# kjedrzejewski/video-cycle_gan-upscaling

Measured on AMD Instinct MI355X. Metric: upscaled frames/s (train step, G+D fwd+bwd) at 256->512, higher is better.
Workload: dtype f32; 1 GPU; C2: make_upscaler_orig((512,512,3),k=3,x2,res=9) + PatchGAN-70, batch 8/GPU, gan2 wiring, Wasserstein + pixel-MSE, faithful 3-call step incl. predict pass; global_batch=8, frame=256x256->512x512, parallelism=dp1, launch=hipGraph replay

## Files before the change

video-cycle_gan-upscaling_amd/csrc/conv_transpose.hip:

```cpp
#include "vcg_common.hpp"
#include <type_traits>

namespace {

struct ConvTParams {
    const float* x;
    const float* w;
    float* y;
    const float* bias;
    const float* prelu;
    const float* residual;
    int n, cin, h, w_, cout, oh, ow;
    int tiles_x, tiles_y, co_blocks;
    int act;
    float alpha;
};

constexpr int phase_of(int k, int cb) { return (((k - cb) % 2) + 2) % 2; }
constexpr int d_of(int k, int cb) { return (k - cb - phase_of(k, cb)) / 2; }
constexpr int dmin_of(int K, int cb) { int m = 1000; for (int k = 0; k < K; ++k) m = d_of(k, cb) < m ? d_of(k, cb) : m; return m; }
constexpr int dmax_of(int K, int cb) { int m = -1000; for (int k = 0; k < K; ++k) m = d_of(k, cb) > m ? d_of(k, cb) : m; return m; }

template <int K, int CBY, int CBX, int CK, int MT>
struct ConvTCfg {
    static constexpr int QROWS = 4;
    static constexpr int DMINY = dmin_of(K, CBY), DMAXY = dmax_of(K, CBY);
    static constexpr int DMINX = dmin_of(K, CBX), DMAXX = dmax_of(K, CBX);
    static constexpr int NDY = DMAXY - DMINY + 1, NDX = DMAXX - DMINX + 1;
    static constexpr int NR = QROWS + DMAXY - DMINY;
    static constexpr int NC = 32 + DMAXX - DMINX;
    static constexpr int PLANE = NR * NC;
    static constexpr int T = K * K;
    static constexpr int IN_ELEMS = CK * PLANE;
    static constexpr int MB = 32 * MT;
    static constexpr int W_ELEMS = CK * T * MB;
    static constexpr int IN_PT = (IN_ELEMS + 255) / 256;
    static constexpr int W_PT = (W_ELEMS + 255) / 256;
    static constexpr size_t LDS_BYTES = (size_t)(IN_ELEMS + W_ELEMS) * sizeof(float);
};

template <int K, int CBY, int CBX, int CK, int MT>
__global__ __launch_bounds__(256, (MT == 1 ? 2 : 1)) void convt_kernel(const ConvTParams p) {
    using C = ConvTCfg<K, CBY, CBX, CK, MT>;
    extern __shared__ __attribute__((aligned(16))) float smem[];
    float* s_in = smem;
    float* s_w = smem + C::IN_ELEMS;

    const int tid = threadIdx.x, lane = tid & 63, wv = tid >> 6;
    const int half = lane >> 5, l31 = lane & 31;
    int b = blockIdx.x;
    const int cb = b % p.co_blocks; b /= p.co_blocks;
    const int tx = b % p.tiles_x;   b /= p.tiles_x;
    const int ty = b % p.tiles_y;   b /= p.tiles_y;
    const int n = b;
    const int qx0 = tx * 32, qy0 = ty * C::QROWS, co0 = cb * C::MB;
    const int gy0 = qy0 - C::DMAXY, gx0 = qx0 - C::DMAXX;
    const float* xn = p.x + (size_t)n * p.cin * p.h * p.w_;

    float rin[C::IN_PT], rw[C::W_PT];
    unsigned in_off[C::IN_PT];
#pragma unroll
    for (int i = 0; i < C::IN_PT; ++i) {
        const int e = tid + i * 256;
        unsigned off = VCG_OOB;
        if (e < C::IN_ELEMS) {
            const int ci = e / C::PLANE, rem = e % C::PLANE;
            const int r = rem / C::NC, c = rem % C::NC;
            const int gy = gy0 + r, gx = gx0 + c;
            if (gy >= 0 && gy < p.h && gx >= 0 && gx < p.w_) off = 4u * (unsigned)((ci * p.h + gy) * p.w_ + gx);
        }
        in_off[i] = off;
    }
    const int hw = p.h * p.w_;
    unsigned w_off[C::W_PT];
#pragma unroll
    for (int i = 0; i < C::W_PT; ++i) {
        const int e = tid + i * 256;
        const int m = e % C::MB, q = e / C::MB;
        const int t = q % C::T, ci = q / C::T;
        const int col = co0 + m < p.cout ? co0 + m : p.cout - 1;
        w_off[i] = e < C::W_ELEMS ? 4u * (unsigned)((t * p.cin + ci) * p.cout + col) : VCG_OOB;
    }
    const size_t wbytes = (size_t)C::T * p.cin * p.cout * sizeof(float);
    auto load_chunk = [&](int ci0) {
        const vcg_rsrc rx = make_rsrc(xn + (size_t)ci0 * hw, (size_t)(p.cin - ci0) * hw * sizeof(float));
#pragma unroll
        for (int i = 0; i < C::IN_PT; ++i) rin[i] = buf_load(rx, in_off[i]);
        const vcg_rsrc rwt = make_rsrc(p.w + (size_t)ci0 * p.cout, wbytes - (size_t)ci0 * p.cout * sizeof(float));
#pragma unroll
        for (int i = 0; i < C::W_PT; ++i) rw[i] = buf_load(rwt, w_off[i]);
    };
    auto store_chunk = [&]() {
#pragma unroll
        for (int i = 0; i < C::IN_PT; ++i) {
            const int e = tid + i * 256;
            if (e < C::IN_ELEMS) s_in[e] = rin[i];
        }
#pragma unroll
        for (int i = 0; i < C::W_PT; ++i) {
            const int e = tid + i * 256;
            if (e < C::W_ELEMS) s_w[e] = rw[i];
        }
    };

    f32x16 acc[2][2][MT];
#pragma unroll
    for (int a = 0; a < 2; ++a)
#pragma unroll
        for (int c = 0; c < 2; ++c)
#pragma unroll
            for (int m = 0; m < MT; ++m)
#pragma unroll
                for (int r = 0; r < 16; ++r) acc[a][c][m][r] = 0.f;

    const float* bbase = s_in + half * C::PLANE + wv * C::NC + l31;
    const float* abase = s_w + half * C::T * C::MB + l31;

    const int nchunks = (p.cin + CK - 1) / CK;
    load_chunk(0);
    for (int c = 0; c < nchunks; ++c) {
        __syncthreads();
        store_chunk();
        __syncthreads();
        if (c + 1 < nchunks) load_chunk((c + 1) * CK);
#pragma unroll
        for (int cp = 0; cp < CK / 2; ++cp) {
            float bv[C::NDY][C::NDX];
#pragma unroll
            for (int iy = 0; iy < C::NDY; ++iy)
#pragma unroll
                for (int ix = 0; ix < C::NDX; ++ix)
                    bv[iy][ix] = bbase[cp * 2 * C::PLANE + (C::DMAXY - (C::DMINY + iy)) * C::NC +
                                       (C::DMAXX - (C::DMINX + ix))];
            float av[C::T][MT];
#pragma unroll
            for (int t = 0; t < C::T; ++t)
#pragma unroll
                for (int mt = 0; mt < MT; ++mt) av[t][mt] = abase[(cp * 2 * C::T + t) * C::MB + mt * 32];
#pragma unroll
            for (int ky = 0; ky < K; ++ky) {
#pragma unroll
                for (int kx = 0; kx < K; ++kx) {
                    const int t = ky * K + kx;
                    const int py = phase_of(ky, CBY), px = phase_of(kx, CBX);
                    const int iy = d_of(ky, CBY) - C::DMINY, ix = d_of(kx, CBX) - C::DMINX;
#pragma unroll
                    for (int mt = 0; mt < MT; ++mt) acc[py][px][mt] = mfma32(av[t][mt], bv[iy][ix], acc[py][px][mt]);
                }
            }
        }
    }

    const int qy = qy0 + wv, qx = qx0 + l31;
    const bool vec_ok = (p.ow % 2) == 0;
    const bool full = vec_ok && (co0 + C::MB <= p.cout) && (2 * (qy0 + C::QROWS) <= p.oh) && (2 * (qx0 + 32) <= p.ow);
    const int plane = p.oh * p.ow;
    const size_t img = (size_t)n * p.cout * plane;
    float* yimg = p.y + img;
    const float* rimg = p.residual ? p.residual + img : nullptr;
    const int ob = (co0 + 4 * half) * plane + (2 * qy) * p.ow + 2 * qx;
    const float* bp = p.bias ? p.bias : vcg_zero_word;
    const int bmask = p.bias ? ~0 : 0;
    const bool is_prelu = p.act == VCG_ACT_PRELU;
    const float* ap = is_prelu ? p.prelu : vcg_zero_word;
    const int amask = is_prelu ? ~0 : 0;
    const float slope_u = (p.act == VCG_ACT_LRELU) ? p.alpha : 1.f;
    auto emit = [&](auto guard_tag, auto res_tag) {
        constexpr bool GUARD = decltype(guard_tag)::value, RES = decltype(res_tag)::value;
#pragma unroll
        for (int mt = 0; mt < MT; ++mt) {
#pragma unroll
            for (int r = 0; r < 16; ++r) {
                const int row = mt * 32 + mfma_row(r, lane);
                const int co = co0 + row;
                const bool co_ok = !GUARD || co < p.cout;
                const int cs = co_ok ? co : co0;
                const float bvv = bp[cs & bmask];
                const float pa = ap[cs & amask];
                const float al = is_prelu ? pa : slope_u;
#pragma unroll
                for (int py = 0; py < 2; ++py) {
                    const int o = ob + (row - 4 * half) * plane + py * p.ow;
                    float v0 = acc[py][0][mt][r] + bvv, v1 = acc[py][1][mt][r] + bvv;
                    v0 = v0 >= 0.f ? v0 : v0 * al;
                    v1 = v1 >= 0.f ? v1 : v1 * al;
                    if (!GUARD) {
                        if (RES) { const float2 rr = *reinterpret_cast<const float2*>(rimg + o); v0 += rr.x; v1 += rr.y; }
                        *reinterpret_cast<float2*>(yimg + o) = make_float2(v0, v1);
                    } else {
                        const int oy = 2 * qy + py, ox = 2 * qx;
                        if (co_ok && oy < p.oh && ox < p.ow) {
                            if (vec_ok) {
                                if (RES) { const float2 rr = *reinterpret_cast<const float2*>(rimg + o); v0 += rr.x; v1 += rr.y; }
                                *reinterpret_cast<float2*>(yimg + o) = make_float2(v0, v1);
                            } else {
                                if (RES) v0 += rimg[o];
                                yimg[o] = v0;
                                if (ox + 1 < p.ow) {
                                    if (RES) v1 += rimg[o + 1];
                                    yimg[o + 1] = v1;
                                }
                            }
                        }
                    }
                }
            }
        }
    };
    using T_ = std::true_type;
    using F_ = std::false_type;
    if (full) {
        if (p.residual) emit(F_{}, T_{}); else emit(F_{}, F_{});
    } else {
        if (p.residual) emit(T_{}, T_{}); else emit(T_{}, F_{});
    }
}

template <int K, int CBY, int CBX, int CK, int MT>
int launch_convt(ConvTParams p, hipStream_t st) {
    using C = ConvTCfg<K, CBY, CBX, CK, MT>;
    p.tiles_x = ceil_div(ceil_div(p.ow, 2), 32);
    p.tiles_y = ceil_div(ceil_div(p.oh, 2), C::QROWS);
    p.co_blocks = ceil_div(p.cout, C::MB);
    const long grid = (long)p.tiles_x * p.tiles_y * p.co_blocks * p.n;
    if (grid <= 0 || grid > 0x7fffffffL) return VCG_E_SHAPE;
    auto kern = convt_kernel<K, CBY, CBX, CK, MT>;
    if (int e = vcg_allow_dyn_lds(reinterpret_cast<const void*>(kern), C::LDS_BYTES)) return e;
    hipLaunchKernelGGL(kern, dim3((int)grid), dim3(256), C::LDS_BYTES, st, p);
    VCG_LAUNCH_CHECK();
    return VCG_OK;
}

}

int vcg_internal_convt(const float* x, const float* w, float* y, int n, int cin, int h, int wd, int cout,
                       int oh, int ow, int k, int cby, int cbx, const vcg_epilogue* ep, hipStream_t st) {
    ConvTParams p{};
    p.x = x; p.w = w; p.y = y;
    p.bias = ep ? ep->bias : nullptr;
    p.prelu = ep ? ep->prelu_alpha : nullptr;
    p.residual = ep ? ep->residual : nullptr;
    p.act = ep ? ep->act : VCG_ACT_NONE;
    p.alpha = ep ? ep->act_alpha : 0.f;
    if (p.act == VCG_ACT_PRELU && p.prelu == nullptr) return VCG_E_NULL;
    if (p.act == VCG_ACT_TANH) return VCG_E_UNSUPPORTED;
    p.n = n; p.cin = cin; p.h = h; p.w_ = wd; p.cout = cout; p.oh = oh; p.ow = ow;
    if (n <= 0 || cin <= 0 || cout <= 0 || oh <= 0 || ow <= 0) return VCG_E_SHAPE;
#define VCG_CT(K_, A_, B_, CK_, MT_) if (k == K_ && cby == A_ && cbx == B_) return launch_convt<K_, A_, B_, CK_, MT_>(p, st)
    VCG_CT(3, 0, 0, 16, 1); VCG_CT(3, 0, 1, 16, 1); VCG_CT(3, 1, 0, 16, 1); VCG_CT(3, 1, 1, 16, 1);
    VCG_CT(4, 1, 1, 16, 1);
    VCG_CT(5, 1, 1, 8, 2); VCG_CT(5, 1, 2, 8, 2); VCG_CT(5, 2, 1, 8, 2); VCG_CT(5, 2, 2, 8, 2);
#undef VCG_CT
    return VCG_E_UNSUPPORTED;
}
```

Before: 138.4 frames/s.

## Add persistent double-buffered transposed-conv kernel for K=3 with small cin

Adds a persistent transposed-convolution kernel launched with one workgroup per CU. Each workgroup keeps its 32-output-channel weight slice resident in LDS and walks a strided sequence of spatial tiles. It prefetches the next input chunk, or the next tile's first chunk, into registers while MFMAs run on a double-buffered LDS input. The goal is to amortize weight loads and hide global-load latency across tiles for the 3x3 upscaler layers with cin<=64. The cost is low occupancy (one 512-thread block per CU) and possible load imbalance across the persistent grid.

```diff
diff --git a/video-cycle_gan-upscaling_amd/csrc/conv_transpose.hip b/video-cycle_gan-upscaling_amd/csrc/conv_transpose.hip
--- a/video-cycle_gan-upscaling_amd/csrc/conv_transpose.hip
+++ b/video-cycle_gan-upscaling_amd/csrc/conv_transpose.hip
@@ -216,9 +216,297 @@
     }
 }
 
+template <int K, int CBY, int CBX, int CK, int MAXC>
+struct ConvTPCfg {
+    static constexpr int QROWS = 8, NT = 64 * QROWS;
+    static constexpr int DMINY = dmin_of(K, CBY), DMAXY = dmax_of(K, CBY);
+    static constexpr int DMINX = dmin_of(K, CBX), DMAXX = dmax_of(K, CBX);
+    static constexpr int NDY = DMAXY - DMINY + 1, NDX = DMAXX - DMINX + 1;
+    static constexpr int NR = QROWS + DMAXY - DMINY;
+    static constexpr int NC = 32 + DMAXX - DMINX;
+    static constexpr int PLANE = NR * NC;
+    static constexpr int T = K * K;
+    static constexpr int IN_ELEMS = CK * PLANE;
+    static constexpr int IN_PT = (IN_ELEMS + NT - 1) / NT;
+    static constexpr int W_ELEMS = MAXC * T * 32;
+    static constexpr int W_PT = W_ELEMS / NT;
+    static constexpr size_t LDS_BYTES = (size_t)(2 * IN_ELEMS + W_ELEMS) * sizeof(float);
+    static_assert(NC < 256 && W_ELEMS % NT == 0 && MAXC % CK == 0 && CK % 2 == 0, "packed (row, column) of a halo element; whole weight rows per pass");
+    static_assert(LDS_BYTES <= 160 * 1024, "one workgroup a CU");
+};
+
+template <int K, int CBY, int CBX, int CK, int MAXC>
+__global__ __launch_bounds__(512, 1) void convt_persistent_kernel(const ConvTParams p) {
+    using C = ConvTPCfg<K, CBY, CBX, CK, MAXC>;
+    extern __shared__ __attribute__((aligned(16))) float smem[];
+    float* s_in = smem;
+    float* s_w = smem + 2 * C::IN_ELEMS;
+
+    const int tid = threadIdx.x, lane = tid & 63, wv = tid >> 6;
+    const int half = lane >> 5, l31 = lane & 31;
+    const int nblk = p.co_blocks, step = (int)gridDim.x / nblk;
+    const int cb = (int)blockIdx.x % nblk, co0 = cb * 32;
+    const int t0 = (int)blockIdx.x / nblk;
+    const int tiles = p.n * p.tiles_y * p.tiles_x;
+    if (t0 >= tiles) return;
+    const int my_tiles = (tiles - t0 + step - 1) / step;
+    int tx = t0 % p.tiles_x, ty = (t0 / p.tiles_x) % p.tiles_y, n = t0 / (p.tiles_x * p.tiles_y);
+    const int dtx = step % p.tiles_x, dty = (step / p.tiles_x) % p.tiles_y, dn = step / (p.tiles_x * p.tiles_y);
+
+    const int hw = p.h * p.w_;
+    const unsigned w4 = 4u * (unsigned)p.w_, hw4 = 4u * (unsigned)hw;
+    unsigned rel[C::IN_PT], rc[C::IN_PT];
+#pragma unroll
+    for (int i = 0; i < C::IN_PT; ++i) {
+        const int e = tid + i * C::NT;
+        const int ci = e / C::PLANE, rem = e % C::PLANE;
+        const int r = rem / C::NC, c = rem % C::NC;
+        rel[i] = (unsigned)ci * hw4 + (unsigned)r * w4 + 4u * (unsigned)c;
+        rc[i] = (unsigned)(r << 8 | c);
+        asm volatile("" : "+v"(rc[i]));
+    }
+    const bool last_live = tid + (C::IN_PT - 1) * C::NT < C::IN_ELEMS;
+    unsigned voff[C::IN_PT];
+    auto tile_offsets = [&](int ty_, int tx_) {
+        const int gy0 = ty_ * C::QROWS - C::DMAXY, gx0 = tx_ * 32 - C::DMAXX;
+        const unsigned tb = (unsigned)gy0 * w4 + 4u * (unsigned)gx0;
+#pragma unroll
+        for (int i = 0; i < C::IN_PT; ++i) {
+            bool ok = (unsigned)(gy0 + (int)(rc[i] >> 8)) < (unsigned)p.h && (unsigned)(gx0 + (int)(rc[i] & 255u)) < (unsigned)p.w_;
+            if (i == C::IN_PT - 1) ok = ok && last_live;
+            voff[i] = ok ? tb + rel[i] : VCG_OOB;
+        }
+    };
+    float rin[C::IN_PT];
+    auto load_chunk = [&](int n_, int ci0) {
+        const vcg_rsrc rx = make_rsrc(p.x + ((size_t)n_ * p.cin + ci0) * hw, (size_t)(p.cin - ci0) * hw * sizeof(float));
+#pragma unroll
+        for (int i = 0; i < C::IN_PT; ++i) rin[i] = buf_load(rx, voff[i]);
+    };
+    auto store_chunk = [&](float* buf) {
+#pragma unroll
+        for (int i = 0; i < C::IN_PT; ++i) {
+            const int e = tid + i * C::NT;
+            if (e < C::IN_ELEMS) buf[e] = rin[i];
+        }
+    };
+    tile_offsets(ty, tx);
+    load_chunk(n, 0);
+
+    {
+        const vcg_rsrc rwt = make_rsrc(p.w, (size_t)C::T * p.cin * p.cout * sizeof(float));
+        const unsigned col = co0 + l31 < p.cout ? 4u * (unsigned)(co0 + l31) : VCG_OOB;
+        float rw[C::W_PT];
+#pragma unroll
+        for (int i = 0; i < C::W_PT; ++i) {
+            const int q = (tid >> 5) + (C::NT / 32) * i;
+            const int ci = q / C::T, tt = q % C::T;
+            const unsigned row = ci < p.cin ? 4u * (unsigned)((tt * p.cin + ci) * p.cout) : VCG_OOB;
+            rw[i] = buf_load(rwt, __builtin_elementwise_add_sat(col, row));
+        }
+#pragma unroll
+        for (int i = 0; i < C::W_PT; ++i) s_w[tid + i * C::NT] = rw[i];
+    }
+    store_chunk(s_in);
+    lds_barrier();
+
+    const unsigned plane = (unsigned)(p.oh * p.ow), plane4 = 4u * plane, ow4 = 4u * (unsigned)p.ow;
+    const int nch = p.cout - co0 < 32 ? p.cout - co0 : 32;
+    const size_t blk_bytes = (size_t)nch * plane * sizeof(float);
+    const bool is_prelu = p.act == VCG_ACT_PRELU;
+    const float slope_u = (p.act == VCG_ACT_LRELU) ? p.alpha : 1.f;
+    const bool vec_ok = (p.ow % 2) == 0;
+    const vcg_rsrc rbias = make_rsrc(p.bias, p.bias ? (size_t)p.cout * sizeof(float) : 0);
+    const vcg_rsrc rslope = make_rsrc(is_prelu ? p.prelu : nullptr, is_prelu ? (size_t)p.cout * sizeof(float) : 0);
+    const unsigned chan4 = 4u * (unsigned)(co0 + 4 * half);
+    auto epilogue = [&](f32x16 (&acc)[2][2], int n_, int qy0, int qx0) {
+        const size_t blk = ((size_t)n_ * p.cout + co0) * plane;
+        const vcg_rsrc ry = make_rsrc(p.y + blk, blk_bytes);
+        const vcg_rsrc rr = make_rsrc(p.residual ? p.residual + blk : nullptr, p.residual ? blk_bytes : 0);
+        const int oy = 2 * (qy0 + wv), ox = 2 * (qx0 + l31);
+        const unsigned base = (unsigned)(4 * half) * plane4 + (unsigned)oy * ow4 + 4u * (unsigned)ox;
+        unsigned vo[2], vo1[2];
+#pragma unroll
+        for (int py = 0; py < 2; ++py) {
+            vo[py] = (oy + py < p.oh && ox < p.ow) ? base + (unsigned)py * ow4 : VCG_OOB;
+            vo1[py] = (oy + py < p.oh && ox + 1 < p.ow) ? base + (unsigned)py * ow4 + 4u : VCG_OOB;
+        }
+        auto emit = [&](auto vec_tag, auto res_tag) {
+            constexpr bool VEC = decltype(vec_tag)::value, RES = decltype(res_tag)::value;
+            constexpr int RG = 4, NG = 16 / RG;
+            float rs[2][RG][2][2];
+            auto srow_of = [&](int r) { return (unsigned)((r & 3) + 8 * (r >> 2)) * plane4; };
+            auto load_res = [&](int g) {
+#pragma unroll
+                for (int j = 0; j < RG; ++j) {
+                    const unsigned srow = srow_of(g * RG + j);
+#pragma unroll
+                    for (int py = 0; py < 2; ++py) {
+                        if (VEC) {
+                            const u32x2 q = __builtin_amdgcn_raw_buffer_load_b64(rr, (int)__builtin_elementwise_add_sat(vo[py], srow), 0, 0);
+                            rs[g & 1][j][py][0] = __uint_as_float(q.x);
+                            rs[g & 1][j][py][1] = __uint_as_float(q.y);
+                        } else {
+                            rs[g & 1][j][py][0] = buf_load(rr, __builtin_elementwise_add_sat(vo[py], srow));
+                            rs[g & 1][j][py][1] = buf_load(rr, __builtin_elementwise_add_sat(vo1[py], srow));
+                        }
+                    }
+                }
+            };
+            if (RES) load_res(0);
+#pragma unroll
+            for (int g = 0; g < NG; ++g) {
+                float bvg[RG], alg[RG];
+#pragma unroll
+                for (int j = 0; j < RG; ++j) {
+                    const int r = g * RG + j;
+                    const unsigned c4 = chan4 + 4u * (unsigned)((r & 3) + 8 * (r >> 2));
+                    bvg[j] = buf_load(rbias, c4);
+                    const float pa = buf_load(rslope, c4);
+                    alg[j] = is_prelu ? pa : slope_u;
+                }
+                if (RES && g + 1 < NG) load_res(g + 1);
+#pragma unroll
+                for (int j = 0; j < RG; ++j) {
+                    const int r = g * RG + j;
+                    const unsigned srow = srow_of(r);
+                    const float bvv = bvg[j], al = alg[j];
+#pragma unroll
+                    for (int py = 0; py < 2; ++py) {
+                        float v0 = acc[py][0][r] + bvv, v1 = acc[py][1][r] + bvv;
+                        v0 = v0 >= 0.f ? v0 : v0 * al;
+                        v1 = v1 >= 0.f ? v1 : v1 * al;
+                        if (RES) { v0 += rs[g & 1][j][py][0]; v1 += rs[g & 1][j][py][1]; }
+                        if (VEC) {
+                            const u32x2 q = {__float_as_uint(v0), __float_as_uint(v1)};
+                            __builtin_amdgcn_raw_buffer_store_b64(q, ry, (int)__builtin_elementwise_add_sat(vo[py], srow), 0, 0);
+                        } else {
+                            buf_store(ry, __builtin_elementwise_add_sat(vo[py], srow), v0);
+                            buf_store(ry, __builtin_elementwise_add_sat(vo1[py], srow), v1);
+                        }
+                    }
+                }
+            }
+        };
+        using T_ = std::true_type;
+        using F_ = std::false_type;
+        if (vec_ok) {
+            if (p.residual) emit(T_{}, T_{}); else emit(T_{}, F_{});
+        } else {
+            if (p.residual) emit(F_{}, T_{}); else emit(F_{}, F_{});
+        }
+    };
+
+    const float* bbase = s_in + half * C::PLANE + wv * C::NC + l31;
+    const float* abase = s_w + half * C::T * 32 + l31;
+    const int nchunks = (p.cin + CK - 1) / CK;
+    int cur = 0;
+    for (int it = 0; it < my_tiles; ++it) {
+        const bool more = it + 1 < my_tiles;
+        const int n0 = n, qy0 = ty * C::QROWS, qx0 = tx * 32;
+
+        f32x16 acc[2][2];
+#pragma unroll
+        for (int a = 0; a < 2; ++a)
+#pragma unroll
+            for (int c = 0; c < 2; ++c)
+#pragma unroll
+                for (int r = 0; r < 16; ++r) acc[a][c][r] = 0.f;
+
+        for (int c = 0; c < nchunks; ++c) {
+            const bool last = c + 1 == nchunks;
+            if (!last) {
+                load_chunk(n0, (c + 1) * CK);
+            } else if (more) {
+                tx += dtx;
+                const int cx = tx >= p.tiles_x ? 1 : 0;
+                tx -= cx ? p.tiles_x : 0;
+                ty += dty + cx;
+                const int cy = ty >= p.tiles_y ? 1 : 0;
+                ty -= cy ? p.tiles_y : 0;
+                n += dn + cy;
+                tile_offsets(ty, tx);
+                load_chunk(n, 0);
+            }
+
+            const float* bb = bbase + cur * C::IN_ELEMS;
+            const float* ab = abase + c * (CK * C::T * 32);
+            float bv[2][C::NDY][C::NDX], av[2][C::T];
+            auto rd = [&](int cp, int s) {
+#pragma unroll
+                for (int iy = 0; iy < C::NDY; ++iy)
+#pragma unroll
+                    for (int ix = 0; ix < C::NDX; ++ix)
+                        bv[s][iy][ix] = bb[cp * 2 * C::PLANE + (C::DMAXY - (C::DMINY + iy)) * C::NC + (C::DMAXX - (C::DMINX + ix))];
+#pragma unroll
+                for (int t = 0; t < C::T; ++t) av[s][t] = ab[(cp * 2 * C::T + t) * 32];
+            };
+            rd(0, 0);
+#pragma unroll
+            for (int cp = 0; cp < CK / 2; ++cp) {
+                const int s = cp & 1;
+                if (cp + 1 < CK / 2) rd(cp + 1, s ^ 1);
+#pragma unroll
+                for (int ky = 0; ky < K; ++ky) {
+#pragma unroll
+                    for (int kx = 0; kx < K; ++kx) {
+                        const int py = phase_of(ky, CBY), px = phase_of(kx, CBX);
+                        const int iy = d_of(ky, CBY) - C::DMINY, ix = d_of(kx, CBX) - C::DMINX;
+                        acc[py][px] = mfma32(av[s][ky * K + kx], bv[s][iy][ix], acc[py][px]);
+                    }
+                }
+                if (cp + 1 < CK / 2) __builtin_amdgcn_sched_group_barrier(0x100, C::NDY * C::NDX + C::T, 0);
+                __builtin_amdgcn_sched_group_barrier(0x008, C::T, 0);
+            }
+            if (!last || more) {
+                store_chunk(s_in + (cur ^ 1) * C::IN_ELEMS);
+                lds_barrier();
+                cur ^= 1;
+            }
+        }
+        epilogue(acc, n0, qy0, qx0);
+    }
+}
+
+bool convt_block_fits(int oh, int ow, int ck, int h, int w) {
+    const unsigned long long lim = 0xFFFFFFE0ull;
+    return 32ull * oh * ow * sizeof(float) < lim && (unsigned long long)ck * h * w * sizeof(float) < lim;
+}
+
+int convt_cu_count() {
+    static const int cus = [] {
+        int dev = 0, v = 0;
+        if (hipGetDevice(&dev) != hipSuccess || hipDeviceGetAttribute(&v, hipDeviceAttributeMultiprocessorCount, dev) != hipSuccess) return 0;
+        return v;
+    }();
+    return cus;
+}
+
+template <int K, int CBY, int CBX, int CK, int MAXC>
+int launch_convt_persistent(ConvTParams p, hipStream_t st) {
+    using C = ConvTPCfg<K, CBY, CBX, CK, MAXC>;
+    if (!convt_block_fits(p.oh, p.ow, CK, p.h, p.w_)) return VCG_E_UNSUPPORTED;
+    p.tiles_x = ceil_div(ceil_div(p.ow, 2), 32);
+    p.tiles_y = ceil_div(ceil_div(p.oh, 2), C::QROWS);
+    p.co_blocks = ceil_div(p.cout, 32);
+    const long tiles = (long)p.tiles_x * p.tiles_y * p.co_blocks * p.n;
+    if (tiles <= 0 || tiles > 0x7fffffffL) return VCG_E_SHAPE;
+    const int cus = convt_cu_count();
+    if (cus <= 0) return VCG_E_UNSUPPORTED;
+    long grid = tiles < (long)cus ? tiles : (long)cus;
+    grid -= grid % p.co_blocks;
+    if (grid < p.co_blocks) grid = p.co_blocks;
+    auto kern = convt_persistent_kernel<K, CBY, CBX, CK, MAXC>;
+    if (int e = vcg_allow_dyn_lds(reinterpret_cast<const void*>(kern), C::LDS_BYTES)) return e;
+    hipLaunchKernelGGL(kern, dim3((int)grid), dim3(C::NT), C::LDS_BYTES, st, p);
+    VCG_LAUNCH_CHECK();
+    return VCG_OK;
+}
+
 template <int K, int CBY, int CBX, int CK, int MT>
 int launch_convt(ConvTParams p, hipStream_t st) {
     using C = ConvTCfg<K, CBY, CBX, CK, MT>;
+    if (!convt_block_fits(p.oh, p.ow, CK, p.h, p.w_)) return VCG_E_UNSUPPORTED;
     p.tiles_x = ceil_div(ceil_div(p.ow, 2), 32);
     p.tiles_y = ceil_div(ceil_div(p.oh, 2), C::QROWS);
     p.co_blocks = ceil_div(p.cout, C::MB);
@@ -246,6 +534,9 @@
     if (p.act == VCG_ACT_TANH) return VCG_E_UNSUPPORTED;
     p.n = n; p.cin = cin; p.h = h; p.w_ = wd; p.cout = cout; p.oh = oh; p.ow = ow;
     if (n <= 0 || cin <= 0 || cout <= 0 || oh <= 0 || ow <= 0) return VCG_E_SHAPE;
+#define VCG_CTP(K_, A_, B_) if (k == K_ && cby == A_ && cbx == B_ && cin <= 64) return launch_convt_persistent<K_, A_, B_, 16, 64>(p, st)
+    VCG_CTP(3, 0, 0); VCG_CTP(3, 0, 1); VCG_CTP(3, 1, 0); VCG_CTP(3, 1, 1);
+#undef VCG_CTP
 #define VCG_CT(K_, A_, B_, CK_, MT_) if (k == K_ && cby == A_ && cbx == B_) return launch_convt<K_, A_, B_, CK_, MT_>(p, st)
     VCG_CT(3, 0, 0, 16, 1); VCG_CT(3, 0, 1, 16, 1); VCG_CT(3, 1, 0, 16, 1); VCG_CT(3, 1, 1, 16, 1);
     VCG_CT(4, 1, 1, 16, 1);
```

Measured after the change: 138.6 frames/s (median of 5 runs). No clear change (+0.1%).
